# SamsungSAILMontreal/ghn3

Measured on AMD Instinct MI355X. Metric: predicted-params/sec (GHN fwd+bwd), ghn3xlm16, 256-node graphs, higher is better.
Workload: dtype f16; 1 GPU; ghn3xlm16 fwd+bwd, 1 synthetic 256-node graph(s) per GPU (seed 256000+), 86515016 predicted params per GPU, loss = sum of Frobenius norms of the predicted tensors; ghn_params=654365312, decoder_rows=1421, workspace_bytes=2436048640, zero_fill_bytes=2797339192, parallelism=dp1, index_mode=reference, loss=fused into the tile kernels

## Files before the change

ghn3_amd/csrc/elementwise.hip:

```cpp

#include "ghn3_internal.h"

#define MAX_DEGREE 100
#define MAX_INPUT_DIST 1000

__device__ __forceinline__ float wsum(float v) {
#pragma unroll
    for (int o = 32; o > 0; o >>= 1) v += __shfl_xor(v, o, 64);
    return v;
}

static int launch_ok(const char* what) {
    hipError_t e = hipGetLastError();
    if (e != hipSuccess) { ghn3_set_error("%s launch: %s", what, hipGetErrorString(e)); return GHN3_E_HIP; }
    return GHN3_OK;
}

__global__ __launch_bounds__(256) void graph_prologue_kernel(const int64_t* __restrict__ A, int* __restrict__ deg_in,
                                                             int* __restrict__ deg_out, int* __restrict__ dist0,
                                                             int* __restrict__ pair, int N, int V) {
    __shared__ int red[2][4];
    const int i = blockIdx.x, b = blockIdx.y;
    const int64_t* Ab = A + (size_t)b * N * N;
    int cnt_out = 0, cnt_in = 0;
// ... 703 lines not shown
                                                       float* __restrict__ b_parts) {
    extern __shared__ float tl[];
    float ss = 0.f, bm = 0.f;
    const int64_t di_raw = blocks[2 * (size_t)blockIdx.x];
    if (di_raw < 0) {
        const ghn3_tile_desc* D = desc + (~di_raw);
        const int64_t word = blocks[2 * (size_t)blockIdx.x + 1];
        const int a0 = (int)(word & 0xffffff), i0 = (int)(word >> 24);
        const int T1 = D->T[1], T3 = D->T[3], hw = D->T[2] * T3, E1 = D->E[1];
        const int ni = min(D->_pad, T1 - i0);
        const float* src = srcs.p[D->src_buf] + D->src_off + (int64_t)(a0 % D->E[0]) * D->S[0];
        const int n = ni * hw;
        const int S2 = (int)D->S[2], S3 = (int)D->S[3];
        const float inv_ni = 1.f / (float)ni, inv_t3 = 1.f / (float)T3;
        const bool vec = E1 == T1 && (ni & 3) == 0 && (S2 & 3) == 0 && (S3 & 3) == 0 &&
                         ((reinterpret_cast<uintptr_t>(src + i0)) & 15) == 0;
        if (vec) {
            const int ni4 = ni >> 2, n4 = ni4 * hw;
            const float inv_ni4 = 1.f / (float)ni4;
            constexpr int U = 4;
            for (int b0 = threadIdx.x; b0 < n4; b0 += 256 * U) {
                float4 v[U];
                int li[U];
#pragma unroll
                for (int u = 0; u < U; ++u) {
                    const int idx = b0 + 256 * u;
                    int pp = (int)((float)idx * inv_ni4);
                    int i4 = idx - pp * ni4;
                    if (i4 < 0) { i4 += ni4; --pp; } else if (i4 >= ni4) { i4 -= ni4; ++pp; }
                    int y = (int)((float)pp * inv_t3);
                    int x = pp - y * T3;
                    if (x < 0) { x += T3; --y; } else if (x >= T3) { x -= T3; ++y; }
                    li[u] = i4 * 4 * hw + pp;
                    v[u] = idx < n4 ? *reinterpret_cast<const float4*>(src + (int64_t)y * S2 + (int64_t)x * S3 + i0 + i4 * 4)
                                    : make_float4(0.f, 0.f, 0.f, 0.f);
                }
#pragma unroll
                for (int u = 0; u < U; ++u)
                    if (b0 + 256 * u < n4) {
                        tl[li[u]] = v[u].x; tl[li[u] + hw] = v[u].y; tl[li[u] + 2 * hw] = v[u].z; tl[li[u] + 3 * hw] = v[u].w;
                    }
            }
        } else {
            constexpr int U = 8;
            for (int b0 = threadIdx.x; b0 < n; b0 += 256 * U) {
                float v[U];
                int li[U];
#pragma unroll
                for (int u = 0; u < U; ++u) {
                    const int idx = b0 + 256 * u;
                    int pp = (int)((float)idx * inv_ni);
                    int i = idx - pp * ni;
                    if (i < 0) { i += ni; --pp; } else if (i >= ni) { i -= ni; ++pp; }
                    int y = (int)((float)pp * inv_t3);
                    int x = pp - y * T3;
                    if (x < 0) { x += T3; --y; } else if (x >= T3) { x -= T3; ++y; }
                    li[u] = i * hw + pp;
                    const int si = i0 + i;
                    v[u] = idx < n ? src[(int64_t)y * S2 + (int64_t)x * S3 + (E1 == T1 ? si : si % E1)] : 0.f;
                }
#pragma unroll
                for (int u = 0; u < U; ++u)
                    if (b0 + 256 * u < n) tl[li[u]] = v[u];
            }
        }
        __syncthreads();
        float* dst = flat + D->dst_off + ((int64_t)a0 * T1 + i0) * hw;
        const float scale = D->scale;
        const int nv = n & ~3;
        for (int j = threadIdx.x * 4; j < nv; j += 1024) {
            f4u o;
            o.x = tl[j] * scale; o.y = tl[j + 1] * scale; o.z = tl[j + 2] * scale; o.w = tl[j + 3] * scale;
            *reinterpret_cast<f4u*>(dst + j) = o;
            ss += (o.x * o.x + o.y * o.y) + (o.z * o.z + o.w * o.w);
            bm = fmaxf(fmaxf(bm, fmaxf(fabsf(o.x), fabsf(o.y))), fmaxf(fabsf(o.z), fabsf(o.w)));
        }
        for (int j = nv + threadIdx.x; j < n; j += 256) { const float o = tl[j] * scale; dst[j] = o; ss += o * o; bm = fmaxf(bm, fabsf(o)); }
        if (sq_parts) tile_block_sumsq(ss, bm, sq_parts, b_parts, D);
        return;
    }
    const int64_t di = di_raw;
    const unsigned start = (unsigned)blocks[2 * (size_t)blockIdx.x + 1];
    const ghn3_tile_desc* D = desc + di;
    const int T0 = D->T[0], T1 = D->T[1], T2 = D->T[2], T3 = D->T[3];
    const unsigned numel = (unsigned)T0 * T1 * T2 * T3;
    const unsigned end = min(numel, start + TILE_CHUNK);
    const float* src = srcs.p[D->src_buf] + D->src_off;
    float* dst = flat + D->dst_off;
    const int E0 = D->E[0], E1 = D->E[1], E2 = D->E[2], E3 = D->E[3];
    const bool w0 = E0 != T0, w1 = E1 != T1, w2 = E2 != T2, w3 = E3 != T3;
    const int S0 = (int)D->S[0], S1 = (int)D->S[1], S2 = (int)D->S[2], S3 = (int)D->S[3];
    const int mode = D->mode;
    const float scale = D->scale;
    Odo o;
    unsigned e = start + threadIdx.x;
    o.init(e, 256, T0, T1, T2, T3);
#pragma unroll 2
    for (; e < end; e += 256) {
        const int m0 = w0 ? o.d[0] % E0 : o.d[0];
        const int m1 = w1 ? o.d[1] % E1 : o.d[1];
        const int m2 = w2 ? o.d[2] % E2 : o.d[2];
        const int m3 = w3 ? o.d[3] % E3 : o.d[3];
        const int64_t so = (int64_t)m0 * S0 + (int64_t)m1 * S1 + (int64_t)m2 * S2 + (int64_t)m3 * S3;
        const float val = norm_apply(src[so], mode, scale);
        dst[e] = val;
        ss += val * val;
        bm = fmaxf(bm, fabsf(val));
        o.step();
    }
    if (sq_parts) tile_block_sumsq(ss, bm, sq_parts, b_parts, D);
}

int ghn3_tile_fwd(float* flat, const float* const* srcs, const ghn3_tile_desc* d_desc, int n_desc, int64_t total,
                  const int64_t* blocks, int lds_bytes, float* sq_parts, float* b_parts, hipStream_t s) {
    if (n_desc <= 0 || total <= 0) return GHN3_OK;
    SrcTable st;
    for (int i = 0; i < 6; ++i) st.p[i] = srcs[i];
    if (lds_bytes > 48 * 1024) {
        if (lds_bytes > 128 * 1024) { ghn3_set_error("tile_fwd: row blocks need %d bytes of LDS", lds_bytes); return GHN3_E_LIMIT; }
        hipFuncSetAttribute((const void*)tile_fwd_kernel, hipFuncAttributeMaxDynamicSharedMemorySize, lds_bytes);
    }
    hipLaunchKernelGGL(tile_fwd_kernel, dim3((unsigned)total), dim3(256), lds_bytes, s, flat, st, d_desc, blocks, sq_parts,
                       sq_parts ? b_parts : nullptr);
    return launch_ok("tile_fwd");
}

template <int U>
__device__ __forceinline__ void tile_bwd_gather(const float* __restrict__ p, int b0, int lim, f4u (&acc)[U]) {
#pragma unroll
    for (int u = 0; u < U; ++u) {
        const int j = b0 + 1024 * u;
        if (j + 4 <= lim) {
            acc[u] += *reinterpret_cast<const f4u*>(p + j);
        } else {
            if (j < lim) acc[u].x += p[j];
            if (j + 1 < lim) acc[u].y += p[j + 1];
            if (j + 2 < lim) acc[u].z += p[j + 2];
        }
    }
}
struct NormLoss { const float* out; const float* norms; const int* desc_seg; const float* g; };
struct H16 { const int64_t* tab; int bf16; };
__device__ __forceinline__ unsigned short h16_cast(float x, int bf16) {
    if (bf16) {
        const unsigned u = __float_as_uint(x);
        return (unsigned short)((u + 0x7fffu + ((u >> 16) & 1u)) >> 16);
    }
    return __builtin_bit_cast(unsigned short, (_Float16)x);
}
__device__ __forceinline__ int64_t h16_index(unsigned rel, unsigned ld32, unsigned ld16) {
    const unsigned r = rel / ld32;
    return (int64_t)r * ld16 + (rel - r * ld32);
}
__global__ __launch_bounds__(256) void tile_bwd_kernel(const float* __restrict__ dflat, SrcTable srcs, DstTable dsrcs,
                                                       const ghn3_tile_desc* __restrict__ desc,
                                                       const int64_t* __restrict__ blocks, float* __restrict__ amax,
                                                       NormLoss nl_, H16 h16) {
    extern __shared__ float tl[];
    float mx = 0.f;
    const int64_t di_raw = blocks[2 * (size_t)blockIdx.x];
    const int64_t di_any = di_raw < 0 ? ~di_raw : di_raw;
    float kn = 0.f;
    if (nl_.norms) {
        const float nrm = nl_.norms[nl_.desc_seg[di_any]];
        kn = nrm > 0.f ? nl_.g[0] / nrm : 0.f;
    }
    unsigned short* hdst = nullptr;
    unsigned hrel0 = 0, hld32 = 1, hld16 = 0;
    float hsc = 1.f;
    if (h16.tab) {
        const float bnd = nl_.norms[-1] * fabsf(nl_.g[0]);
        if (blockIdx.x == 0 && threadIdx.x == 0 && amax) amax[0] = bnd;
        const int64_t h = h16.tab[3 * di_any];
        if (h != INT64_MIN && desc[di_any].src_buf == 0) {
            hdst = reinterpret_cast<unsigned short*>(dsrcs.p[0]) + h;
            hrel0 = (unsigned)h16.tab[3 * di_any + 1];
            const int64_t lds_ = h16.tab[3 * di_any + 2];
            hld32 = (unsigned)(lds_ & 0xffffffff); hld16 = (unsigned)(lds_ >> 32);
            hsc = ghn3_pow2_scale(bnd);
        }
    }
    const float* __restrict__ outp = nl_.norms ? nl_.out + desc[di_any].dst_off : nullptr;
    if (di_raw < 0) {
        const ghn3_tile_desc* D = desc + (~di_raw);
        const int64_t word = blocks[2 * (size_t)blockIdx.x + 1];
        const int a0 = (int)(word & 0xffffff), i0 = (int)(word >> 24);
        const int T0 = D->T[0], T1 = D->T[1], T3 = D->T[3], hw = D->T[2] * T3;
        const int E0 = D->E[0], E1 = D->E[1], R1 = D->R[1];
        const int ni = min(D->_pad, R1 - i0);
        const int nl = max(0, min(ni, E1 - i0));
        float* dsrc = dsrcs.p[D->src_buf] + D->src_off + (int64_t)a0 * D->S[0] + i0;
        const float* g = dflat ? dflat + D->dst_off : nullptr;
        const bool live = a0 < E0 && nl > 0;
        if (live) {
            const int n = nl * hw;
            constexpr int U = 4;
            for (int b0 = threadIdx.x * 4; b0 < n; b0 += 1024 * U) {
                f4u acc[U], acc2[U];
#pragma unroll
                for (int u = 0; u < U; ++u) { acc[u] = f4u{0.f, 0.f, 0.f, 0.f}; acc2[u] = f4u{0.f, 0.f, 0.f, 0.f}; }
                for (int t0 = a0; t0 < T0; t0 += E0)
                    for (int r0 = 0; r0 + i0 < T1; r0 += E1) {
                        const int lim = min(nl, T1 - r0 - i0) * hw;
                        const int64_t go = ((int64_t)t0 * T1 + r0 + i0) * hw;
                        if (g) tile_bwd_gather<U>(g + go, b0, lim, acc);
                        if (outp) tile_bwd_gather<U>(outp + go, b0, lim, acc2);
                    }
                if (outp) {
#pragma unroll
                    for (int u = 0; u < U; ++u) {
                        acc[u].x += kn * acc2[u].x; acc[u].y += kn * acc2[u].y; acc[u].z += kn * acc2[u].z; acc[u].w += kn * acc2[u].w;
                    }
                }
#pragma unroll
                for (int u = 0; u < U; ++u) {
                    const int j = b0 + 1024 * u;
                    if (j + 4 <= n) {
                        *reinterpret_cast<float4*>(tl + j) = make_float4(acc[u].x, acc[u].y, acc[u].z, acc[u].w);
                    } else {
                        if (j < n) tl[j] = acc[u].x;
                        if (j + 1 < n) tl[j + 1] = acc[u].y;
                        if (j + 2 < n) tl[j + 2] = acc[u].z;
                    }
                }
            }
            __syncthreads();
        }
        const float scale = D->scale;
        const int S2 = (int)D->S[2], S3 = (int)D->S[3];
        const float inv_t3 = 1.f / (float)T3;
        if ((ni & 3) == 0 && (S2 & 3) == 0 && (S3 & 3) == 0 && (reinterpret_cast<uintptr_t>(dsrc) & 15) == 0) {
            const int ni4 = ni >> 2, nw4 = ni4 * hw;
            const float inv_ni4 = 1.f / (float)ni4;
            for (int idx = threadIdx.x; idx < nw4; idx += 256) {
                int pp = (int)((float)idx * inv_ni4);
                int i4 = idx - pp * ni4;
                if (i4 < 0) { i4 += ni4; --pp; } else if (i4 >= ni4) { i4 -= ni4; ++pp; }
                int y = (int)((float)pp * inv_t3);
                int x = pp - y * T3;
                if (x < 0) { x += T3; --y; } else if (x >= T3) { x -= T3; ++y; }
                const int i = i4 * 4;
                float4 val;
                val.x = (live && i < nl) ? tl[i * hw + pp] * scale : 0.f;
                val.y = (live && i + 1 < nl) ? tl[(i + 1) * hw + pp] * scale : 0.f;
                val.z = (live && i + 2 < nl) ? tl[(i + 2) * hw + pp] * scale : 0.f;
                val.w = (live && i + 3 < nl) ? tl[(i + 3) * hw + pp] * scale : 0.f;
                if (hdst) {
                    unsigned short* hp = hdst + h16_index(hrel0 + (unsigned)(a0 * (int)D->S[0] + i0 + y * S2 + x * S3 + i), hld32, hld16);
                    us4h o;
                    o[0] = h16_cast(val.x * hsc, h16.bf16); o[1] = h16_cast(val.y * hsc, h16.bf16);
                    o[2] = h16_cast(val.z * hsc, h16.bf16); o[3] = h16_cast(val.w * hsc, h16.bf16);
                    if ((reinterpret_cast<uintptr_t>(hp) & 7) == 0) *reinterpret_cast<us4h*>(hp) = o;
                    else { hp[0] = o[0]; hp[1] = o[1]; hp[2] = o[2]; hp[3] = o[3]; }
                    continue;
                }
                *reinterpret_cast<float4*>(dsrc + (int64_t)y * S2 + (int64_t)x * S3 + i) = val;
                mx = fmaxf(fmaxf(mx, fmaxf(fabsf(val.x), fabsf(val.y))), fmaxf(fabsf(val.z), fabsf(val.w)));
            }
        } else {
            const float inv_ni = 1.f / (float)ni;
            const int nw = ni * hw;
            for (int idx = threadIdx.x; idx < nw; idx += 256) {
                int pp = (int)((float)idx * inv_ni);
                int i = idx - pp * ni;
                if (i < 0) { i += ni; --pp; } else if (i >= ni) { i -= ni; ++pp; }
                int y = (int)((float)pp * inv_t3);
                int x = pp - y * T3;
                if (x < 0) { x += T3; --y; } else if (x >= T3) { x -= T3; ++y; }
                const float val = (live && i < nl) ? tl[i * hw + pp] * scale : 0.f;
                if (hdst) {
                    hdst[h16_index(hrel0 + (unsigned)(a0 * (int)D->S[0] + i0 + y * S2 + x * S3 + i), hld32, hld16)] = h16_cast(val * hsc, h16.bf16);
                    continue;
                }
                dsrc[(int64_t)y * S2 + (int64_t)x * S3 + i] = val;
                mx = fmaxf(mx, fabsf(val));
            }
        }
        if (amax && D->src_buf == 0 && !h16.tab) ghn3_atomic_amax(amax, mx);
        return;
    }
    const int64_t di = di_raw;
    const unsigned start = (unsigned)blocks[2 * (size_t)blockIdx.x + 1];
    const ghn3_tile_desc* D = desc + di;
    const int R0 = D->R[0], R1 = D->R[1], R2 = D->R[2], R3 = D->R[3];
    const unsigned numel = (unsigned)R0 * R1 * R2 * R3;
    const unsigned end = min(numel, start + TILE_CHUNK);
    const float* src = srcs.p[D->src_buf] + D->src_off;
    float* dsrc = dsrcs.p[D->src_buf] + D->src_off;
    const float* g = dflat ? dflat + D->dst_off : nullptr;
    const int T0 = D->T[0], T1 = D->T[1], T2 = D->T[2], T3 = D->T[3];
    const int E0 = D->E[0], E1 = D->E[1], E2 = D->E[2], E3 = D->E[3];
    const int S0 = (int)D->S[0], S1 = (int)D->S[1], S2 = (int)D->S[2], S3 = (int)D->S[3];
    const int mode = D->mode;
    const float scale = D->scale;
    Odo o;
    unsigned e = start + threadIdx.x;
    o.init(e, 256, R0, R2, R3, R1);
    for (; e < end; e += 256) {
        const int a0 = o.d[0], a2 = o.d[1], a3 = o.d[2], a1 = o.d[3];
        const int64_t so = (int64_t)a0 * S0 + (int64_t)a1 * S1 + (int64_t)a2 * S2 + (int64_t)a3 * S3;
        float acc = 0.f, acc2 = 0.f;
        if (a0 < E0 && a1 < E1 && a2 < E2 && a3 < E3) {
            for (int t0 = a0; t0 < T0; t0 += E0)
                for (int t1 = a1; t1 < T1; t1 += E1)
                    for (int t2 = a2; t2 < T2; t2 += E2)
                        for (int t3 = a3; t3 < T3; t3 += E3) {
                            const int64_t gi = (((int64_t)t0 * T1 + t1) * T2 + t2) * T3 + t3;
                            if (g) acc += g[gi];
                            if (outp) acc2 += outp[gi];
                        }
            acc = (acc + kn * acc2) * norm_grad(src[so], mode, scale);
        }
        if (hdst) hdst[h16_index(hrel0 + (unsigned)so, hld32, hld16)] = h16_cast(acc * hsc, h16.bf16);
        else dsrc[so] = acc;
        mx = fmaxf(mx, fabsf(acc));
        o.step();
    }
    if (amax && D->src_buf == 0 && !h16.tab) ghn3_atomic_amax(amax, mx);
}

int ghn3_tile_bwd(const float* dflat, const float* const* srcs, float* const* dsrcs, const ghn3_tile_desc* d_desc,
                  int n_desc, int64_t total, const int64_t* blocks, int lds_bytes, float* amax, const float* out,
                  const float* norms, const int* desc_seg, const float* gscale, const int64_t* h16_tab, int h16_bf16,
                  hipStream_t s) {
    if (n_desc <= 0 || total <= 0) return GHN3_OK;
    if (!dflat && !norms) { ghn3_set_error("tile_bwd: neither an upstream gradient nor the fused norm loss"); return GHN3_E_ARG; }
    if (norms && (!out || !desc_seg || !gscale)) { ghn3_set_error("tile_bwd: the fused norm loss needs out, the descriptor -> tensor table and g"); return GHN3_E_ARG; }
    if (h16_tab && (dflat || !norms || !amax)) { ghn3_set_error("tile_bwd: direct 16-bit tiles need the fused norm loss alone (no upstream gradient) and the amax slot"); return GHN3_E_ARG; }
    NormLoss nl{out, norms, desc_seg, gscale};
    H16 h16{h16_tab, h16_bf16};
    SrcTable st; DstTable dt;
    for (int i = 0; i < 6; ++i) { st.p[i] = srcs[i]; dt.p[i] = dsrcs[i]; }
    if (lds_bytes > 48 * 1024) {
        if (lds_bytes > 128 * 1024) { ghn3_set_error("tile_bwd: row blocks need %d bytes of LDS", lds_bytes); return GHN3_E_LIMIT; }
        hipFuncSetAttribute((const void*)tile_bwd_kernel, hipFuncAttributeMaxDynamicSharedMemorySize, lds_bytes);
    }
    hipLaunchKernelGGL(tile_bwd_kernel, dim3((unsigned)total), dim3(256), lds_bytes, s, dflat, st, dt, d_desc, blocks,
                       amax, nl, h16);
    return launch_ok("tile_bwd");
}

#define NORM_CHUNK 8192
__device__ __forceinline__ int first_segment_after(const int64_t* __restrict__ seg_off, int n_seg, int64_t pos) {
    int lo = 0, hi = n_seg;
    while (lo < hi) {
        const int mid = (lo + hi) >> 1;
        if (seg_off[2 * mid + 1] > pos) hi = mid; else lo = mid + 1;
    }
    return lo;
}
__global__ __launch_bounds__(256) void param_sq_kernel(const float* __restrict__ flat,
                                                       const int64_t* __restrict__ seg_off, float* __restrict__ norms,
                                                       int n_seg, const int* __restrict__ first_seg,
                                                       float* __restrict__ parts) {
    __shared__ float red[4];
    const int64_t w0 = (int64_t)blockIdx.x * NORM_CHUNK, w1 = w0 + NORM_CHUNK;
    const int sg0 = first_seg ? first_seg[blockIdx.x] : first_segment_after(seg_off, n_seg, w0);
    for (int sgm = sg0; sgm < n_seg && seg_off[2 * sgm] < w1; ++sgm) {
        const int64_t c0 = max(seg_off[2 * sgm], w0), c1 = min(seg_off[2 * sgm + 1], w1);
        float acc = 0.f;
        const int64_t a0 = (c0 + 3) & ~(int64_t)3, a1 = c1 & ~(int64_t)3;
        if (a0 < a1) {
            const float4* f4 = reinterpret_cast<const float4*>(flat + a0);
            const int64_t n4 = (a1 - a0) >> 2;
            for (int64_t q = threadIdx.x; q < n4; q += 256) {
                const float4 v = f4[q];
                acc += v.x * v.x + v.y * v.y + v.z * v.z + v.w * v.w;
            }
            for (int64_t e = c0 + threadIdx.x; e < a0; e += 256) { const float v = flat[e]; acc += v * v; }
            for (int64_t e = a1 + threadIdx.x; e < c1; e += 256) { const float v = flat[e]; acc += v * v; }
        } else {
            for (int64_t e = c0 + threadIdx.x; e < c1; e += 256) { const float v = flat[e]; acc += v * v; }
        }
        acc = wsum(acc);
        __syncthreads();
        if ((threadIdx.x & 63) == 0) red[threadIdx.x >> 6] = acc;
        __syncthreads();
        if (threadIdx.x == 0) {
            const float t = (red[0] + red[1]) + (red[2] + red[3]);
            if (parts && first_seg) parts[sg0 + (int64_t)blockIdx.x + (sgm - sg0)] = t;
            else if (t != 0.f) atomicAdd(&norms[sgm], t);
        }
    }
}
__global__ __launch_bounds__(256) void param_sqrt_kernel(float* __restrict__ norms, int n_seg,
                                                         const int64_t* __restrict__ seg_off,
                                                         const int* __restrict__ first_seg,
                                                         const float* __restrict__ parts) {
    const int i = blockIdx.x * 4 + (threadIdx.x >> 6), lane = threadIdx.x & 63;
    if (i >= n_seg) return;
    float sq = 0.f;
    if (parts && first_seg) {
        if (seg_off[2 * i + 1] > seg_off[2 * i]) {
            const int64_t b0 = seg_off[2 * i] / NORM_CHUNK, b1 = (seg_off[2 * i + 1] - 1) / NORM_CHUNK;
            for (int64_t b = b0 + lane; b <= b1; b += 64) sq += parts[b + i];
        }
        sq = wsum(sq);
    } else {
        sq = norms[i];
    }
    if (lane == 0) norms[i] = sqrtf(sq);
}
__global__ void param_loss_kernel(float* __restrict__ loss, const float* __restrict__ norms, int n_seg) {
    __shared__ float tot[256];
    float acc = 0.f;
    for (int i = threadIdx.x; i < n_seg; i += 256) acc += norms[i];
    tot[threadIdx.x] = acc;
    __syncthreads();
    if (threadIdx.x == 0) {
        float t = 0.f;
        for (int k = 0; k < 256; ++k) t += tot[k];
        loss[0] += t;
    }
}
__global__ __launch_bounds__(256) void param_norm_fin_kernel(float* __restrict__ norms, int n_seg,
                                                             const float* __restrict__ parts,
                                                             const int* __restrict__ first,
                                                             const float* __restrict__ b_parts, float* __restrict__ ratio) {
    const int i = blockIdx.x * 4 + (threadIdx.x >> 6), lane = threadIdx.x & 63;
    if (i >= n_seg) return;
    float sq = 0.f, bm = 0.f;
    for (int b = first[i] + lane; b < first[i + 1]; b += 64) { sq += parts[b]; if (b_parts) bm = fmaxf(bm, b_parts[b]); }
    sq = wsum(sq);
#pragma unroll
    for (int o = 32; o > 0; o >>= 1) bm = fmaxf(bm, __shfl_xor(bm, o, 64));
    if (lane == 0) {
        const float nrm = sqrtf(sq);
        norms[i] = nrm;
        if (ratio) ratio[i] = nrm > 0.f ? bm / nrm : 0.f;
    }
}
__global__ void param_loss_set_kernel(float* __restrict__ loss, const float* __restrict__ norms, int n_seg,
                                      const float* __restrict__ ratio, float* __restrict__ bound) {
    __shared__ float tot[256], mx[256];
    float acc = 0.f, m = 0.f;
    for (int i = threadIdx.x; i < n_seg; i += 256) { acc += norms[i]; if (ratio) m = fmaxf(m, ratio[i]); }
    tot[threadIdx.x] = acc;
    mx[threadIdx.x] = m;
    __syncthreads();
    if (threadIdx.x == 0) {
        float t = 0.f, b = 0.f;
        for (int k = 0; k < 256; ++k) { t += tot[k]; b = fmaxf(b, mx[k]); }
        loss[0] = t;
        if (bound) bound[0] = b;
    }
}
int ghn3_param_norm_fin(float* loss, float* norms, const float* parts, const int* first, int n_seg, const float* b_parts,
                        float* ratio, float* bound, hipStream_t s) {
    if (n_seg <= 0) return GHN3_OK;
    if (b_parts && !(ratio && bound)) { ghn3_set_error("PARAM_NORM_FIN: bound parts need the ratio scratch (r5) and the bound slot (r6)"); return GHN3_E_ARG; }
    if (!b_parts) ratio = nullptr, bound = nullptr;
    hipLaunchKernelGGL(param_norm_fin_kernel, dim3((n_seg + 3) / 4), dim3(256), 0, s, norms, n_seg, parts, first, b_parts, ratio);
    hipLaunchKernelGGL(param_loss_set_kernel, dim3(1), dim3(256), 0, s, loss, norms, n_seg, ratio, bound);
    return launch_ok("param_norm_fin");
}

int ghn3_param_norm_fwd(float* loss, const float* flat, const int64_t* seg_off, float* norms, int n_seg,
                        int64_t flat_numel, const int* first_seg, float* parts, hipStream_t s) {
    if (n_seg <= 0) return GHN3_OK;
    if (!(parts && first_seg)) hipMemsetAsync(norms, 0, sizeof(float) * n_seg, s);
    const int64_t blocks = (flat_numel + NORM_CHUNK - 1) / NORM_CHUNK;
    hipLaunchKernelGGL(param_sq_kernel, dim3((unsigned)blocks), dim3(256), 0, s, flat, seg_off, norms, n_seg,
                       first_seg, parts);
    hipLaunchKernelGGL(param_sqrt_kernel, dim3((n_seg + 3) / 4), dim3(256), 0, s, norms, n_seg, seg_off, first_seg, parts);
    hipLaunchKernelGGL(param_loss_kernel, dim3(1), dim3(256), 0, s, loss, norms, n_seg);
    return launch_ok("param_norm_fwd");
}
__global__ __launch_bounds__(256) void param_norm_bwd_kernel(float* __restrict__ dflat, const float* __restrict__ flat,
                                                             const int64_t* __restrict__ seg_off,
                                                             const float* __restrict__ norms, int n_seg, float g,
                                                             const int* __restrict__ first_seg) {
    const int64_t w0 = (int64_t)blockIdx.x * NORM_CHUNK, w1 = w0 + NORM_CHUNK;
    for (int sgm = first_seg ? first_seg[blockIdx.x] : first_segment_after(seg_off, n_seg, w0);
         sgm < n_seg && seg_off[2 * sgm] < w1; ++sgm) {
        const int64_t c0 = max(seg_off[2 * sgm], w0), c1 = min(seg_off[2 * sgm + 1], w1);
        const float nrm = norms[sgm];
        const float k = nrm > 0.f ? g / nrm : 0.f;
        const int64_t a0 = (c0 + 3) & ~(int64_t)3, a1 = c1 & ~(int64_t)3;
        if (a0 < a1) {
            const float4* f4 = reinterpret_cast<const float4*>(flat + a0);
            float4* d4 = reinterpret_cast<float4*>(dflat + a0);
            const int64_t n4 = (a1 - a0) >> 2;
            for (int64_t q = threadIdx.x; q < n4; q += 256) {
                float4 v = f4[q];
                v.x *= k; v.y *= k; v.z *= k; v.w *= k;
                d4[q] = v;
            }
            for (int64_t e = c0 + threadIdx.x; e < a0; e += 256) dflat[e] = flat[e] * k;
            for (int64_t e = a1 + threadIdx.x; e < c1; e += 256) dflat[e] = flat[e] * k;
        } else {
            for (int64_t e = c0 + threadIdx.x; e < c1; e += 256) dflat[e] = flat[e] * k;
// ... 901 lines not shown
```

ghn3_amd/csrc/ghn3_internal.h:

```cpp
#pragma once
#include <hip/hip_runtime.h>
#include <stdint.h>
#include "ghn3_hip.h"

struct GemmProbDev {
    const float* A; const float* B; float* C;
    const float* bias; const float* residual; const float* aux_in; float* aux_out;
    const int* a_gather; const int* b_gather; const int* c_gather;
    int M, N, K, lda, ldb, ldc;
    int a_q, a_s, b_q, b_s, c_q, c_s;
    int bias_q, bias_s, bias_stride;
    int act, dact, flags;
    float alpha;
    int tile_start;
    int tiles_m, tiles_n;
    int ksplit, k_chunk;
    int order;
    int kq, ks;
    const int* lim;
    int lim_kind;
    int xcd_cols;
    int pin;
    int pin_first, pin_count;
    int pin_end, pin_total;
    const float* alpha_amax;
    int ln_kind;
    float ln_eps;
    const float* ln_p[6];
    const void* B2;
    const int* mtab;
};


int ghn3_gemm_init();
int ghn3_gemm_launch(const GemmProbDev* d_probs, int n_probs, int total_tiles, int a_mode, int b_mode,
                     int tile, int ctype, hipStream_t stream);

int ghn3_gemm_h16d_launch(const GemmProbDev* d_probs, int n_probs, int total_tiles, int tile, int ctype, int grid_cap,
                          hipStream_t stream);
int ghn3_gemm_p8_init();
int ghn3_gemm_p8_launch(const GemmProbDev* d_probs, int n_probs, int total_tiles, int ctype, int grid_cap,
                        hipStream_t stream);
int ghn3_gemm_p8w_launch(const GemmProbDev* d_probs, int n_probs, int total_tiles, int ctype, int grid_cap,
                         hipStream_t stream);
int ghn3_gemm_p8d_launch(const GemmProbDev* d_probs, int n_probs, int total_tiles, int ctype, int grid_cap,
                         hipStream_t stream);
int ghn3_gemm_x3_init();
int ghn3_gemm_x3_tile(int code, int slice, int* bm, int* bn);
int ghn3_gemm_x3_launch(const GemmProbDev* d_probs, int n_probs, int total_tiles, int code, int slice,
                        hipStream_t stream);
int ghn3_gemm_x3s_init();
int ghn3_gemm_x3s_tile(int code, int K, int ln_kind, int* bm, int* bn);
int ghn3_gemm_x3s_launch(const GemmProbDev* d_probs, const GemmProbDev* h_probs, int n_probs, int total_tiles, int code, int K,
                         int ln_kind, hipStream_t stream);
int ghn3_gemm_wg_launch(const GemmProbDev* d_probs, int n_probs, int total_tiles, int grid_cap, int tile_edge, hipStream_t stream);
int ghn3_gemm_small_launch(const GemmProbDev* d_probs, int n_probs, int total_tiles, int a_mode, int b_mode, int with_ln,
                           hipStream_t stream);

int ghn3_attn_init();
int ghn3_attn_fwd(float* out, const float* qkv, const float* bias, float* P, const int* n_nodes,
                  int B, int N, int C, int H, hipStream_t s);
int ghn3_attn_bwd(float* dqkv, const float* dO, const float* qkv, const float* P, const float* O, float* amax_out,
                  float* dBias, const int* n_nodes, int B, int N, int C, int H, int general, hipStream_t s);

int ghn3_graph_prologue(const int64_t* A, int* deg_in, int* deg_out, int* dist0, int* pair,
                        int B, int N, int V, hipStream_t s);
int ghn3_embed_nodes(float* x, const int* node_type, const int* shape_idx, const int* n_nodes, const int* node_off,
                     const float* E_type, const float* E_ch, const float* E_sp, const float* E_in,
                     const float* E_out, const float* E_dist, const int* deg_in, const int* deg_out,
                     const int* dist0, int B, int N, int C, hipStream_t s);
int ghn3_embed_bwd(const float* dx, const int* node_type, const int* shape_idx, const int* n_nodes,
                   const int* node_off, float* dE_type, float* dE_ch, float* dE_sp, float* dE_in, float* dE_out,
                   float* dE_dist, const int* deg_in, const int* deg_out, const int* dist0,
                   int B, int N, int C, int n_type, int n_ch, int n_sp, hipStream_t s);
int ghn3_edge_hidden(float* hid, const float* Pfw, const float* Pbw, int V, int C, hipStream_t s);
int ghn3_edge_hidden_bwd(float* dPfw, float* dPbw, float* dhid, const float* hid, int V, int C, hipStream_t s);
int ghn3_bias_gather(float* bias, const float* T, const int* pair, int B, int N, int H, hipStream_t s);
int ghn3_bias_hist(float* dT, const float* dBias, const int* pair, int B, int N, int H, int V, void* scratch,
                   int have_amax, hipStream_t s);
int ghn3_rowset_colsum(float* out, const float* X, const void* sets, int n_sets, int O, int I, hipStream_t s);
int ghn3_layernorm_fwd(float* y, float* x, const float* g, const float* b, float* mean, float* rstd, const float* add,
                       int n_add, int64_t add_stride, int rows, int C, float eps, hipStream_t s);
int ghn3_layernorm_bwd(float* dx, float* dy, const float* x, const float* g, const float* mean,
                       const float* rstd, const float* res, const float* add, int n_add, int64_t add_stride, int rows,
                       int C, hipStream_t s);
int ghn3_ln_param_grad(float* dg, float* db, const float* dy, const float* x, const float* mean,
                       const float* rstd, int rows, int C, int accum, hipStream_t s);
int ghn3_ln_param_grad_batch(float* gbase, const float* abase, const int64_t* table, int n_items, int rows, int C,
                             hipStream_t s);
int ghn3_tile_fwd(float* flat, const float* const* srcs, const ghn3_tile_desc* d_desc, int n_desc,
                  int64_t total, const int64_t* blocks, int lds_bytes, float* sq_parts, float* b_parts, hipStream_t s);
int ghn3_tile_bwd(const float* dflat, const float* const* srcs, float* const* dsrcs,
                  const ghn3_tile_desc* d_desc, int n_desc, int64_t total, const int64_t* blocks, int lds_bytes,
                  float* amax, const float* out, const float* norms, const int* desc_seg, const float* gscale,
                  const int64_t* h16_tab, int h16_bf16, hipStream_t s);
int ghn3_param_norm_fin(float* loss, float* norms, const float* parts, const int* first, int n_seg, const float* b_parts,
                        float* ratio, float* bound, hipStream_t s);
int ghn3_param_norm_fwd(float* loss, const float* flat, const int64_t* seg_off, float* norms, int n_seg,
                        int64_t flat_numel, const int* first_seg, float* parts, hipStream_t s);
int ghn3_param_norm_bwd(float* dflat, const float* flat, const int64_t* seg_off, const float* norms, int n_seg,
                        float g, int64_t flat_numel, const int* first_seg, hipStream_t s);
int ghn3_colsum(float* out, const float* X, int M, int N, int ld, int q, int sdim, int stride, int accum,
                const int* gather, hipStream_t s);
int ghn3_rowseg_sum(float* out, const float* X, const int* seg_ptr, const int* idx, int rows, int C, int ldx,
                    int ldo, int accum, hipStream_t s);
int ghn3_add(float* dst, const float* src, int64_t n, hipStream_t s);
int ghn3_transpose32(float* dst, const float* src, int rows, int cols, int ld_src, int ld_dst, int batch, int64_t sb, int64_t db,
                     hipStream_t s);
int ghn3_wire_pack(void* dst, const void* src, int64_t n, int64_t n_pad, int reverse, hipStream_t s);
int ghn3_rank_reduce(void* out, const void* in, int64_t per, int W, int in16, int out16, float scale, hipStream_t s);
int ghn3_cast16(const float* src, void* dst, const ghn3_cast_desc* d_desc, int n_desc, int total_blocks, float* dbias,
                const float* amax, int grid_cap, hipStream_t s);
int ghn3_sumsq(float* out, const float* x, int64_t n, float* parts, int64_t skip_lo, int64_t skip_hi, const float* extra,
               int n_extra, hipStream_t s);
int ghn3_adamw(float* p, const float* g, float* m, float* v, int64_t n, const float* sumsq, float lr, float beta1,
               float beta2, float eps, float weight_decay, float bias_corr1, float bias_corr2, float max_norm,
               float inv_scale, hipStream_t s);
int ghn3_adamw_cast16(float* p, const float* g, float* m, float* v, void* dst, const ghn3_cast_desc* d_desc, int n_desc,
                      int total_blocks, const float* sumsq, float lr, float beta1, float beta2, float eps, float weight_decay,
                      float bias_corr1, float bias_corr2, float max_norm, float inv_scale, hipStream_t s);
int ghn3_adamw_s16(float* p, const float* g, void* m, void* v, int64_t n, const float* sumsq, float lr, float beta1,
                   float beta2, float eps, float weight_decay, float bias_corr1, float bias_corr2, float max_norm,
                   float inv_scale, float step, float seed, int64_t base, hipStream_t s);
int ghn3_adamw_s16_cast16(float* p, const float* g, void* m, void* v, void* dst, const ghn3_cast_desc* d_desc, int n_desc,
                          int total_blocks, const float* sumsq, float lr, float beta1, float beta2, float eps,
                          float weight_decay, float bias_corr1, float bias_corr2, float max_norm, float inv_scale, float step,
                          float seed, int64_t base, hipStream_t s);
int ghn3_dact(float* X, const float* aux, int M, int N, int ld, int dact, float* amax, const float* parts, int n_parts,
              int64_t part_stride, int rows_parts, hipStream_t s);

int ghn3_relu_fix(float* X, const float* U, const float* W, const float* bias, int rows, int cols, int ld, int K, int q,
                  int sdim, float tau_rel, hipStream_t s);

void ghn3_set_error(const char* fmt, ...);

#ifdef __HIPCC__
__device__ __forceinline__ int ghn3_amax_exp(float amax) {
    return (int)((__float_as_uint(amax) >> 23) & 0xff) - 127;
}
__device__ __forceinline__ float ghn3_pow2_scale(float amax) {
    const int e = ghn3_amax_exp(amax);
    if (!(amax > 0.f) || e < -100) return 1.f;
    return __uint_as_float((unsigned)(127 + 11 - e) << 23);
}
__device__ __forceinline__ float ghn3_pow2_inv_scale(float amax) {
    const int e = ghn3_amax_exp(amax);
    if (!(amax > 0.f) || e < -100) return 1.f;
    return __uint_as_float((unsigned)(127 - 11 + e) << 23);
}
__device__ __forceinline__ void ghn3_atomic_amax(float* slot, float v) {
#pragma unroll
    for (int o = 32; o > 0; o >>= 1) v = fmaxf(v, __shfl_xor(v, o, 64));
    if ((threadIdx.x & 63) == 0 && v > *reinterpret_cast<volatile float*>(slot))
        atomicMax(reinterpret_cast<int*>(slot), __float_as_int(v));
}
#endif
```

ghn3_amd/csrc/runtime.hip:

```cpp

#include "ghn3_internal.h"
#include <cstdarg>
#include <cstdio>
#include <cstring>
#include <vector>
#include <algorithm>

static thread_local char g_err[512] = "";

void ghn3_set_error(const char* fmt, ...) {
    va_list ap;
    va_start(ap, fmt);
    vsnprintf(g_err, sizeof(g_err), fmt, ap);
    va_end(ap);
}

extern "C" const char* ghn3_last_error(void) { return g_err; }
extern "C" int ghn3_abi_version(void) { return GHN3_ABI_VERSION; }

#define HIPCHK(expr)                                                                  \
    do {                                                                              \
        hipError_t e_ = (expr);                                                       \
        if (e_ != hipSuccess) {                                                       \
            ghn3_set_error("%s failed: %s", #expr, hipGetErrorString(e_));            \
            return GHN3_E_HIP;                                                        \
        }                                                                             \
    } while (0)

static const int kStageSlots = 16;

struct Launch { int a_mode, b_mode, tile, first, count, tiles, with_ln, max_slice; };

struct SlotCache {
    bool valid = false;
    uint64_t stamp = 0;
    int n_ops = 0, n_problems = 0, n_bufs = 0;
    std::vector<ghn3_op> ops;
    std::vector<ghn3_gemm_problem> problems;
    std::vector<void*> bufs;
    std::vector<std::vector<Launch>> launches;
    hipStream_t up_stream = nullptr;
};

struct ghn3_ctx {
    SlotCache* cache;
    uint64_t clock;
    uint64_t cache_hits, cache_misses;
    GemmProbDev* h_stage[kStageSlots];
    GemmProbDev* d_stage[kStageSlots];
    hipEvent_t ev[kStageSlots];
    bool ev_used[kStageSlots];
    size_t cap;
    int ctype;
    int profile;
    double ms[GHN3_OP_KIND_COUNT];
    int64_t launches[GHN3_OP_KIND_COUNT];
    hipEvent_t pe0, pe1;
    std::vector<hipEvent_t>* pool;
    std::vector<int>* pool_tag;
    size_t pool_used;
    double tag_ms[256];
    int64_t tag_n[256];
    hipStream_t side;
    hipEvent_t ev_fork, ev_join, ev_mark[4];
    bool side_enabled;
    bool side_pending;
    bool mark_set[4];
};

static int ctx_reserve(ghn3_ctx* c, size_t n) {
    if (n <= c->cap) return GHN3_OK;
    size_t cap = std::max<size_t>(n, 1024);
    for (int i = 0; i < kStageSlots; ++i) {
        if (c->ev_used[i]) { HIPCHK(hipEventSynchronize(c->ev[i])); c->ev_used[i] = false; }
        if (c->h_stage[i]) HIPCHK(hipHostFree(c->h_stage[i]));
        if (c->d_stage[i]) HIPCHK(hipFree(c->d_stage[i]));
        c->h_stage[i] = nullptr; c->d_stage[i] = nullptr;
        c->cache[i].valid = false;
        c->cache[i].stamp = 0;
        HIPCHK(hipHostMalloc((void**)&c->h_stage[i], cap * sizeof(GemmProbDev), hipHostMallocDefault));
        HIPCHK(hipMalloc((void**)&c->d_stage[i], cap * sizeof(GemmProbDev)));
    }
    c->cap = cap;
    return GHN3_OK;
}

extern "C" int ghn3_ctx_create(ghn3_ctx** out) {
    if (!out) return GHN3_E_ARG;
    int ndev = 0;
    HIPCHK(hipGetDeviceCount(&ndev));
    if (ndev <= 0) { ghn3_set_error("no HIP device"); return GHN3_E_HIP; }
    ghn3_ctx* c = new ghn3_ctx();
    memset(c, 0, sizeof(*c));
    c->pool = new std::vector<hipEvent_t>();
    c->pool_tag = new std::vector<int>();
    c->cache = new SlotCache[kStageSlots];
    for (int i = 0; i < kStageSlots; ++i) HIPCHK(hipEventCreateWithFlags(&c->ev[i], hipEventDisableTiming));
    HIPCHK(hipEventCreate(&c->pe0));
    HIPCHK(hipEventCreate(&c->pe1));
    {
        int least = 0, greatest = 0;
        HIPCHK(hipDeviceGetStreamPriorityRange(&least, &greatest));
        HIPCHK(hipStreamCreateWithPriority(&c->side, hipStreamNonBlocking, least));
    }
    HIPCHK(hipEventCreateWithFlags(&c->ev_fork, hipEventDisableTiming));
    HIPCHK(hipEventCreateWithFlags(&c->ev_join, hipEventDisableTiming));
    for (int i = 0; i < 4; ++i) HIPCHK(hipEventCreateWithFlags(&c->ev_mark[i], hipEventDisableTiming));
    c->side_enabled = !(getenv("GHN3_NO_SIDE_STREAM") && atoi(getenv("GHN3_NO_SIDE_STREAM")) != 0);
    int rc = ghn3_gemm_init();
    if (rc) return rc;
    rc = ghn3_attn_init();
    if (rc) return rc;
    rc = ghn3_gemm_x3_init();
    if (rc) return rc;
    rc = ghn3_gemm_x3s_init();
    if (rc) return rc;
    rc = ghn3_gemm_p8_init();
    if (rc) return rc;
    rc = ctx_reserve(c, 1024);
    if (rc) return rc;
    *out = c;
    return GHN3_OK;
}

extern "C" void ghn3_ctx_destroy(ghn3_ctx* c) {
    if (!c) return;
    for (int i = 0; i < kStageSlots; ++i) {
        if (c->ev_used[i]) hipEventSynchronize(c->ev[i]);
        if (c->h_stage[i]) hipHostFree(c->h_stage[i]);
        if (c->d_stage[i]) hipFree(c->d_stage[i]);
        hipEventDestroy(c->ev[i]);
    }
    hipEventDestroy(c->pe0);
    hipEventDestroy(c->pe1);
    hipStreamSynchronize(c->side);
    hipStreamDestroy(c->side);
    hipEventDestroy(c->ev_fork);
    for (int i = 0; i < 4; ++i) hipEventDestroy(c->ev_mark[i]);
    hipEventDestroy(c->ev_join);
    for (hipEvent_t e : *c->pool) hipEventDestroy(e);
    delete c->pool;
    delete c->pool_tag;
    delete[] c->cache;
    delete c;
}

extern "C" int ghn3_ctx_set_compute_type(ghn3_ctx* c, int ctype) {
    if (!c) return GHN3_E_NOCTX;
    if (ctype < 0 || ctype > 2) { ghn3_set_error("bad compute type %d", ctype); return GHN3_E_ARG; }
    c->ctype = ctype;
    return GHN3_OK;
}

extern "C" int ghn3_profile_enable(ghn3_ctx* c, int mode) {
    if (!c) return GHN3_E_NOCTX;
    c->profile = mode;
    return GHN3_OK;
}
static int drain_pool(ghn3_ctx* c) {
    for (size_t k = 0; k < c->pool_used; ++k) {
        hipEvent_t e0 = (*c->pool)[2 * k], e1 = (*c->pool)[2 * k + 1];
        HIPCHK(hipEventSynchronize(e1));
        float ms = 0.f;
        HIPCHK(hipEventElapsedTime(&ms, e0, e1));
        const int tag = (*c->pool_tag)[k] & 255;
        c->tag_ms[tag] += ms;
        c->tag_n[tag] += 1;
    }
    c->pool_used = 0;
    return GHN3_OK;
}
extern "C" int ghn3_profile_read(ghn3_ctx* c, double* ms, int64_t* launches, int reset) {
    if (!c) return GHN3_E_NOCTX;
    for (int i = 0; i < GHN3_OP_KIND_COUNT; ++i) {
        if (ms) ms[i] = c->ms[i];
        if (launches) launches[i] = c->launches[i];
        if (reset) { c->ms[i] = 0; c->launches[i] = 0; }
    }
    return GHN3_OK;
}
extern "C" int ghn3_profile_read_tags(ghn3_ctx* c, double* ms256, int64_t* n256, int reset) {
    if (!c) return GHN3_E_NOCTX;
    int rc = drain_pool(c);
    if (rc) return rc;
    for (int i = 0; i < 256; ++i) {
        if (ms256) ms256[i] = c->tag_ms[i];
        if (n256) n256[i] = c->tag_n[i];
        if (reset) { c->tag_ms[i] = 0; c->tag_n[i] = 0; }
    }
    return GHN3_OK;
}

struct Resolver {
    void* const* bufs; int n_bufs; bool bad;
    template <typename T> T* get(const ghn3_ref& r) {
        if (r.buf < 0) return nullptr;
        if (r.buf >= n_bufs || bufs[r.buf] == nullptr) { bad = true; return nullptr; }
        return reinterpret_cast<T*>(reinterpret_cast<char*>(bufs[r.buf]) + r.off);
    }
};

static int pick_tile(const ghn3_gemm_problem& p, int forced, int64_t op_t64) {
    if (p.flags & GHN3_GEMM_X3) {
        if (forced == 44 || forced == 45 || p.ln_kind)
            return (forced == 45 ? 7000 : 6000) + 100 * (p.ln_kind & 3) + ((p.K / 64) % 100);
        return 4000 + 10 * (((forced >= 40 && forced <= 42) ? forced : 40) - 40) + p.x3_slice / 64;
    }
    if (p.ln_kind) return 32;
    if (p.flags & GHN3_GEMM_OP16) {
        if (forced == 16 || forced == 24 || forced == 20 || forced == 25 || forced == 29 || forced == 30) return forced;
        if (forced == 28) {
            const bool kmap_ok = p.b_kq == 0 || p.b_kq % 64 == 0 || 64 % p.b_kq == 0;
            return (p.ksplit <= 1 && p.M >= 160 && (p.N & 3) == 0 && kmap_ok && p.a_gather.buf < 0 && p.b_gather.buf < 0 &&
                    p.c_gather.buf < 0) ? 28 : 16;
        }
        const int64_t t256 = (int64_t)((p.M + 255) / 256) * ((p.N + 255) / 256) * (p.ksplit > 1 ? p.ksplit : 1);
        const double eff = ((double)p.M / (((p.M + 255) / 256) * 256.0)) * ((double)p.N / (((p.N + 255) / 256) * 256.0));
        return (t256 >= 200 && eff >= 0.8) ? 24 : 16;
    }
    if (forced == 48 || forced == 49) {
        const bool ok = p.a_mode == GHN3_MODE_COL && p.b_mode == GHN3_MODE_COL && p.ksplit <= 1 && (p.M & 3) == 0 &&
                        (p.N & 3) == 0 && (p.ldc & 3) == 0 && (p.C.off & 15) == 0 && (p.lda & 3) == 0 && (p.ldb & 3) == 0 &&
                        (p.A.off & 15) == 0 && (p.B.off & 15) == 0 && p.a_gather.buf < 0 &&
                        p.b_gather.buf < 0 && p.c_gather.buf < 0 && !p.a_q && !p.b_q && !p.c_q && !p.bias_q &&
                        p.act == GHN3_ACT_NONE && p.dact == GHN3_DACT_NONE && p.residual.buf < 0 && p.aux_out.buf < 0 &&
                        (p.bias.buf < 0 || (p.flags & GHN3_GEMM_BIASGRAD));
        return ok ? forced : 64;
    }
    if (forced == 32 || forced == 64 || forced == 128) return forced;
    const double flops = 2.0 * p.M * p.N * (double)p.K;
    if (p.ksplit <= 1 && op_t64 <= 640 && flops <= 4e9 && p.K <= 8192) return 32;
    const int64_t t128 = (int64_t)((p.M + 127) / 128) * ((p.N + 127) / 128) * (p.ksplit > 1 ? p.ksplit : 1);
    if (p.M >= 96 && p.N >= 96 && t128 >= 192) return 128;
    return 64;
}

static inline bool is16(int tl) { return tl == 16 || tl == 24 || tl == 20 || tl == 25 || tl == 28 || tl == 29 || tl == 30; }

extern "C" int ghn3_run(ghn3_ctx* c, const ghn3_op* ops, int n_ops, const ghn3_gemm_problem* problems, int n_problems,
                        void* const* bufs, int n_bufs, void* stream_) {
    if (!c) return GHN3_E_NOCTX;
    if (n_ops < 0 || (n_ops > 0 && !ops) || n_bufs < 0) { ghn3_set_error("ghn3_run: bad arguments"); return GHN3_E_ARG; }
    hipStream_t stream = (hipStream_t)stream_;
    Resolver R{bufs, n_bufs, false};

    std::vector<std::vector<Launch>> fresh_launches;
    const std::vector<std::vector<Launch>>* launches = &fresh_launches;
    size_t need = 0;
    for (int k = 0; k < n_ops; ++k)
        if (ops[k].kind == GHN3_OP_GEMM) need += (size_t)ops[k].i[1];
    GemmProbDev* hs = nullptr; GemmProbDev* ds = nullptr;
    static const bool use_cache = !(getenv("GHN3_RUN_CACHE") && atoi(getenv("GHN3_RUN_CACHE")) == 0);
    int hit = -1;
    if (need > 0) {
        int rc = ctx_reserve(c, need);
        if (rc) return rc;
        if (n_problems < 0 || (n_problems > 0 && !problems)) { ghn3_set_error("ghn3_run: bad problem table"); return GHN3_E_ARG; }
        for (int i = 0; use_cache && i < kStageSlots && hit < 0; ++i) {
            const SlotCache& e = c->cache[i];
            if (e.valid && e.n_ops == n_ops && e.n_problems == n_problems && e.n_bufs == n_bufs &&
                memcmp(e.bufs.data(), bufs, (size_t)n_bufs * sizeof(void*)) == 0 &&
                memcmp(e.ops.data(), ops, (size_t)n_ops * sizeof(ghn3_op)) == 0 &&
                memcmp(e.problems.data(), problems, (size_t)n_problems * sizeof(ghn3_gemm_problem)) == 0)
                hit = i;
// ... 632 lines not shown
```

Before: 15.13 billion predicted-params/s.

## Compute tile backward from source tensors instead of re-reading the predicted output

Adds a templated tile backward path for the fused-norm-loss, direct-16-bit case. For mode-0 tiles it recomputes the gradient from the source decoder buffer (scaled value times the repeat count times g/norm) rather than gathering the large tiled output tensor. This avoids streaming the full predicted-parameter output back from memory. It adds closed-form repeat counts, vectorised 16-bit stores and an env switch that defaults on, at the cost of more complex indexing and float-based division tricks.

```diff
diff --git a/ghn3_amd/csrc/elementwise.hip b/ghn3_amd/csrc/elementwise.hip
--- a/ghn3_amd/csrc/elementwise.hip
+++ b/ghn3_amd/csrc/elementwise.hip
@@ -879,6 +879,167 @@
     const unsigned r = rel / ld32;
     return (int64_t)r * ld16 + (rel - r * ld32);
 }
+template <int V>
+__device__ __forceinline__ void h16_store(unsigned short* hp, const unsigned short (&o)[V]) {
+    if constexpr (V == 4) {
+        if ((reinterpret_cast<uintptr_t>(hp) & 7) == 0) { *reinterpret_cast<us4h*>(hp) = us4h{o[0], o[1], o[2], o[3]}; return; }
+    }
+#pragma unroll
+    for (int c = 0; c < V; ++c) hp[c] = o[c];
+}
+template <int V>
+__device__ __forceinline__ void load_v(const float* __restrict__ p, float (&v)[V]) {
+    if constexpr (V == 4) { const f4u t = *reinterpret_cast<const f4u*>(p); v[0] = t.x; v[1] = t.y; v[2] = t.z; v[3] = t.w; }
+    else v[0] = p[0];
+}
+static int g_tile_bwd_src = 1;
+int ghn3_elementwise_init() {
+    if (getenv("GHN3_TILE_BWD_SRC")) g_tile_bwd_src = atoi(getenv("GHN3_TILE_BWD_SRC")) != 0;
+    return GHN3_OK;
+}
+template <int V, int U>
+__device__ __forceinline__ void tile_bwd_rows_src(const float* __restrict__ sp, unsigned short* __restrict__ hdst, unsigned hbase,
+                                                  unsigned hld32, unsigned hld16, int bf16, int ni, int nl, int hw, int T3, int S2,
+                                                  int S3, bool live, int n_lo, int n_hi, int thr, float kn, float scale,
+                                                  float hsc) {
+    const int niv = ni / V, nw = niv * hw;
+    const float inv_niv = 1.f / (float)niv, inv_t3 = 1.f / (float)T3;
+    const unsigned r0 = hbase / hld32, c0 = hbase - r0 * hld32;
+    const bool lin = S2 == T3 * S3 && S3 == (int)hld32 && c0 + (unsigned)ni <= hld32;
+    int pp = (int)((float)threadIdx.x * inv_niv);
+    int iv = (int)threadIdx.x - pp * niv;
+    if (iv < 0) { iv += niv; --pp; } else if (iv >= niv) { iv -= niv; ++pp; }
+    int dq = (int)(256.f * inv_niv);
+    int dr = 256 - dq * niv;
+    if (dr < 0) { dr += niv; --dq; } else if (dr >= niv) { dr -= niv; ++dq; }
+    auto step = [&]() {
+        iv += dr; pp += dq;
+        if (iv >= niv) { iv -= niv; ++pp; }
+    };
+    auto offset = [&](int p, int i) {
+        if (lin) return p * S3 + i;
+        int y = (int)((float)p * inv_t3);
+        int x = p - y * T3;
+        if (x < 0) { x += T3; --y; } else if (x >= T3) { x -= T3; ++y; }
+        return y * S2 + x * S3 + i;
+    };
+    auto put = [&](int p, int i, const unsigned short (&o)[V]) {
+        const int64_t at = lin ? (int64_t)(r0 + (unsigned)p) * hld16 + (c0 + (unsigned)i)
+                               : h16_index(hbase + (unsigned)offset(p, i), hld32, hld16);
+        h16_store<V>(hdst + at, o);
+    };
+    if (!live) {
+        unsigned short z[V];
+#pragma unroll
+        for (int c = 0; c < V; ++c) z[c] = h16_cast(0.f * hsc, bf16);
+        for (int idx = threadIdx.x; idx < nw; idx += 256) {
+            put(pp, iv * V, z);
+            step();
+        }
+        return;
+    }
+    if (thr >= ni) { n_lo += n_hi; n_hi = 0; }
+    const int i_last = (nl - 1) / V * V;
+    for (int b0 = threadIdx.x; b0 < nw; b0 += 256 * U) {
+        float v[U][V], a[U][V];
+        int pp_[U], i_[U];
+#pragma unroll
+        for (int u = 0; u < U; ++u) {
+            pp_[u] = pp; i_[u] = iv * V;
+            step();
+        }
+#pragma unroll
+        for (int u = 0; u < U; ++u)
+            load_v<V>(sp + (b0 + 256 * u < nw ? offset(pp_[u], i_[u]) - max(i_[u] - i_last, 0) : 0), v[u]);
+#pragma unroll
+        for (int u = 0; u < U; ++u)
+#pragma unroll
+            for (int c = 0; c < V; ++c) { v[u][c] *= scale; a[u][c] = 0.f; }
+        for (int k = 0; k < n_lo; ++k)
+#pragma unroll
+            for (int u = 0; u < U; ++u)
+#pragma unroll
+                for (int c = 0; c < V; ++c) a[u][c] += v[u][c];
+        if (n_hi > 0) {
+#pragma unroll
+            for (int u = 0; u < U; ++u)
+#pragma unroll
+                for (int c = 0; c < V; ++c) v[u][c] = i_[u] + c < thr ? v[u][c] : 0.f;
+            for (int k = 0; k < n_hi; ++k)
+#pragma unroll
+                for (int u = 0; u < U; ++u)
+#pragma unroll
+                    for (int c = 0; c < V; ++c) a[u][c] += v[u][c];
+        }
+#pragma unroll
+        for (int u = 0; u < U; ++u) {
+            if (b0 + 256 * u >= nw) break;
+            unsigned short o[V];
+#pragma unroll
+            for (int c = 0; c < V; ++c) {
+                const float val = i_[u] + c < nl ? (0.f + kn * a[u][c]) * scale : 0.f;
+                o[c] = h16_cast(val * hsc, bf16);
+            }
+            put(pp_[u], i_[u], o);
+        }
+    }
+}
+template <int V>
+__device__ __forceinline__ void tile_bwd_elems_src(const ghn3_tile_desc* __restrict__ D, const float* __restrict__ src,
+                                                   unsigned short* __restrict__ hdst, unsigned hrel0, unsigned hld32,
+                                                   unsigned hld16, int bf16, unsigned start, unsigned end, float kn, float hsc) {
+    constexpr int U = V == 4 ? 2 : 4;
+    const int R0 = D->R[0], R1 = D->R[1], R2 = D->R[2], R3 = D->R[3];
+    const int T0 = D->T[0], T1 = D->T[1], T2 = D->T[2], T3 = D->T[3];
+    const int E0 = D->E[0], E1 = D->E[1], E2 = D->E[2], E3 = D->E[3];
+    const int S0 = (int)D->S[0], S1 = (int)D->S[1], S2 = (int)D->S[2], S3 = (int)D->S[3];
+    const float scale = D->scale;
+    const unsigned qend = end / V;
+    Odo o;
+    o.init(start / V + threadIdx.x, 256, R0, R2, R3, R1 / V);
+    for (unsigned q0 = start / V + threadIdx.x; q0 < qend; q0 += 256 * U) {
+        float v[U][V];
+        unsigned rel[U];
+        int a1_[U], n023[U];
+#pragma unroll
+        for (int u = 0; u < U; ++u) {
+            const int a0 = o.d[0], a2 = o.d[1], a3 = o.d[2], a1 = o.d[3] * V;
+            const bool valid = q0 + 256 * u < qend;
+            const int64_t so = (int64_t)a0 * S0 + (int64_t)a1 * S1 + (int64_t)a2 * S2 + (int64_t)a3 * S3;
+            rel[u] = hrel0 + (unsigned)so;
+            a1_[u] = a1;
+            int n = 0;
+            if (valid && a0 < E0 && a2 < E2 && a3 < E3) {
+                int c0 = 0, c2 = 0, c3 = 0;
+                for (int t = a0; t < T0; t += E0) ++c0;
+                for (int t = a2; t < T2; t += E2) ++c2;
+                for (int t = a3; t < T3; t += E3) ++c3;
+                n = c0 * c2 * c3;
+            }
+            n023[u] = n;
+            load_v<V>(src + (valid ? so : 0), v[u]);
+            o.step();
+        }
+#pragma unroll
+        for (int u = 0; u < U; ++u) {
+            if (q0 + 256 * u >= qend) break;
+            unsigned short h[V];
+#pragma unroll
+            for (int c = 0; c < V; ++c) {
+                const int a1 = a1_[u] + c;
+                int n = 0;
+                if (a1 < E1) for (int t = a1; t < T1; t += E1) n += n023[u];
+                const float val = norm_apply(v[u][c], 0, scale);
+                float acc2 = 0.f;
+                for (int k = 0; k < n; ++k) acc2 += val;
+                const float acc = n > 0 ? (0.f + kn * acc2) * norm_grad(v[u][c], 0, scale) : 0.f;
+                h[c] = h16_cast(acc * hsc, bf16);
+            }
+            h16_store<V>(hdst + h16_index(rel[u], hld32, hld16), h);
+        }
+    }
+}
+template <bool SRC>
 __global__ __launch_bounds__(256) void tile_bwd_kernel(const float* __restrict__ dflat, SrcTable srcs, DstTable dsrcs,
                                                        const ghn3_tile_desc* __restrict__ desc,
                                                        const int64_t* __restrict__ blocks, float* __restrict__ amax,
@@ -886,26 +1047,80 @@
     extern __shared__ float tl[];
     float mx = 0.f;
     const int64_t di_raw = blocks[2 * (size_t)blockIdx.x];
+    const int64_t blk_word = SRC ? blocks[2 * (size_t)blockIdx.x + 1] : 0;
     const int64_t di_any = di_raw < 0 ? ~di_raw : di_raw;
     float kn = 0.f;
-    if (nl_.norms) {
-        const float nrm = nl_.norms[nl_.desc_seg[di_any]];
-        kn = nrm > 0.f ? nl_.g[0] / nrm : 0.f;
-    }
     unsigned short* hdst = nullptr;
     unsigned hrel0 = 0, hld32 = 1, hld16 = 0;
     float hsc = 1.f;
-    if (h16.tab) {
-        const float bnd = nl_.norms[-1] * fabsf(nl_.g[0]);
-        if (blockIdx.x == 0 && threadIdx.x == 0 && amax) amax[0] = bnd;
-        const int64_t h = h16.tab[3 * di_any];
-        if (h != INT64_MIN && desc[di_any].src_buf == 0) {
+    ghn3_tile_desc dd;
+    if constexpr (SRC) {
+        dd = desc[di_any];
+        const int seg = nl_.desc_seg[di_any];
+        const int64_t h = h16.tab[3 * di_any], rel0 = h16.tab[3 * di_any + 1], lds_ = h16.tab[3 * di_any + 2];
+        const float gs = nl_.g[0], bnd = nl_.norms[-1] * fabsf(gs);
+        const float nrm = nl_.norms[seg];
+        kn = nrm > 0.f ? gs / nrm : 0.f;
+        if (blockIdx.x == 0 && threadIdx.x == 0) amax[0] = bnd;
+        if (h != INT64_MIN && dd.src_buf == 0) {
             hdst = reinterpret_cast<unsigned short*>(dsrcs.p[0]) + h;
-            hrel0 = (unsigned)h16.tab[3 * di_any + 1];
-            const int64_t lds_ = h16.tab[3 * di_any + 2];
+            hrel0 = (unsigned)rel0;
             hld32 = (unsigned)(lds_ & 0xffffffff); hld16 = (unsigned)(lds_ >> 32);
             hsc = ghn3_pow2_scale(bnd);
         }
+    } else {
+        if (nl_.norms) {
+            const float nrm = nl_.norms[nl_.desc_seg[di_any]];
+            kn = nrm > 0.f ? nl_.g[0] / nrm : 0.f;
+        }
+        if (h16.tab) {
+            const float bnd = nl_.norms[-1] * fabsf(nl_.g[0]);
+            if (blockIdx.x == 0 && threadIdx.x == 0 && amax) amax[0] = bnd;
+            const int64_t h = h16.tab[3 * di_any];
+            if (h != INT64_MIN && desc[di_any].src_buf == 0) {
+                hdst = reinterpret_cast<unsigned short*>(dsrcs.p[0]) + h;
+                hrel0 = (unsigned)h16.tab[3 * di_any + 1];
+                const int64_t lds_ = h16.tab[3 * di_any + 2];
+                hld32 = (unsigned)(lds_ & 0xffffffff); hld16 = (unsigned)(lds_ >> 32);
+                hsc = ghn3_pow2_scale(bnd);
+            }
+        }
+    }
+    bool src_local = false;
+    if constexpr (SRC) src_local = hdst && dd.mode == 0;
+    if (src_local && di_raw < 0) {
+        const int a0 = (int)(blk_word & 0xffffff), i0 = (int)(blk_word >> 24);
+        const int T0 = dd.T[0], T1 = dd.T[1], T3 = dd.T[3], hw = dd.T[2] * T3;
+        const int E0 = dd.E[0], E1 = dd.E[1];
+        const int S0 = (int)dd.S[0], S2 = (int)dd.S[2], S3 = (int)dd.S[3];
+        const int ni = min(dd._pad, dd.R[1] - i0);
+        const int nl = max(0, min(ni, E1 - i0));
+        const bool live = a0 < E0 && nl > 0;
+        const int cnt0 = live ? (T0 - a0 + E0 - 1) / E0 : 0;
+        const int c_hi = live ? max(0, (T1 - i0 + E1 - 1) / E1) : 0;
+        const int n_lo = cnt0 * max(c_hi - 1, 0), n_hi = c_hi > 0 ? cnt0 : 0;
+        const int thr = T1 - i0 - (c_hi - 1) * E1;
+        const float* sp = srcs.p[0] + dd.src_off + (int64_t)a0 * S0 + i0;
+        const float* dsrc = dsrcs.p[0] + dd.src_off + (int64_t)a0 * S0 + i0;
+        const unsigned hbase = hrel0 + (unsigned)(a0 * S0 + i0);
+        if ((ni & 3) == 0 && (S2 & 3) == 0 && (S3 & 3) == 0 && (reinterpret_cast<uintptr_t>(dsrc) & 15) == 0)
+            tile_bwd_rows_src<4, 4>(sp, hdst, hbase, hld32, hld16, h16.bf16, ni, nl, hw, T3, S2, S3, live, n_lo, n_hi, thr, kn,
+                                    dd.scale, hsc);
+        else
+            tile_bwd_rows_src<1, 4>(sp, hdst, hbase, hld32, hld16, h16.bf16, ni, nl, hw, T3, S2, S3, live, n_lo, n_hi, thr, kn,
+                                    dd.scale, hsc);
+        return;
+    }
+    if (src_local) {
+        const unsigned start = (unsigned)blk_word;
+        const unsigned numel = (unsigned)dd.R[0] * dd.R[1] * dd.R[2] * dd.R[3];
+        const unsigned end = min(numel, start + TILE_CHUNK);
+        const float* src = srcs.p[0] + dd.src_off;
+        if (dd.S[1] == 1 && (dd.R[1] & 3) == 0 && ((dd.S[0] | dd.S[2] | dd.S[3]) & 3) == 0 && (hrel0 & 3) == 0 && (hld32 & 3) == 0)
+            tile_bwd_elems_src<4>(&dd, src, hdst, hrel0, hld32, hld16, h16.bf16, start, end, kn, hsc);
+        else
+            tile_bwd_elems_src<1>(&dd, src, hdst, hrel0, hld32, hld16, h16.bf16, start, end, kn, hsc);
+        return;
     }
     const float* __restrict__ outp = nl_.norms ? nl_.out + desc[di_any].dst_off : nullptr;
     if (di_raw < 0) {
@@ -921,7 +1136,7 @@
         const bool live = a0 < E0 && nl > 0;
         if (live) {
             const int n = nl * hw;
-            constexpr int U = 4;
+            constexpr int U = SRC ? 1 : 4;
             for (int b0 = threadIdx.x * 4; b0 < n; b0 += 1024 * U) {
                 f4u acc[U], acc2[U];
 #pragma unroll
@@ -1058,12 +1273,12 @@
     H16 h16{h16_tab, h16_bf16};
     SrcTable st; DstTable dt;
     for (int i = 0; i < 6; ++i) { st.p[i] = srcs[i]; dt.p[i] = dsrcs[i]; }
+    const auto kernel = (h16_tab && g_tile_bwd_src) ? tile_bwd_kernel<true> : tile_bwd_kernel<false>;
     if (lds_bytes > 48 * 1024) {
         if (lds_bytes > 128 * 1024) { ghn3_set_error("tile_bwd: row blocks need %d bytes of LDS", lds_bytes); return GHN3_E_LIMIT; }
-        hipFuncSetAttribute((const void*)tile_bwd_kernel, hipFuncAttributeMaxDynamicSharedMemorySize, lds_bytes);
-    }
-    hipLaunchKernelGGL(tile_bwd_kernel, dim3((unsigned)total), dim3(256), lds_bytes, s, dflat, st, dt, d_desc, blocks,
-                       amax, nl, h16);
+        hipFuncSetAttribute((const void*)kernel, hipFuncAttributeMaxDynamicSharedMemorySize, lds_bytes);
+    }
+    hipLaunchKernelGGL(kernel, dim3((unsigned)total), dim3(256), lds_bytes, s, dflat, st, dt, d_desc, blocks, amax, nl, h16);
     return launch_ok("tile_bwd");
 }
 
diff --git a/ghn3_amd/csrc/ghn3_internal.h b/ghn3_amd/csrc/ghn3_internal.h
--- a/ghn3_amd/csrc/ghn3_internal.h
+++ b/ghn3_amd/csrc/ghn3_internal.h
@@ -88,6 +88,7 @@
                        const float* rstd, int rows, int C, int accum, hipStream_t s);
 int ghn3_ln_param_grad_batch(float* gbase, const float* abase, const int64_t* table, int n_items, int rows, int C,
                              hipStream_t s);
+int ghn3_elementwise_init();
 int ghn3_tile_fwd(float* flat, const float* const* srcs, const ghn3_tile_desc* d_desc, int n_desc,
                   int64_t total, const int64_t* blocks, int lds_bytes, float* sq_parts, float* b_parts, hipStream_t s);
 int ghn3_tile_bwd(const float* dflat, const float* const* srcs, float* const* dsrcs,
diff --git a/ghn3_amd/csrc/runtime.hip b/ghn3_amd/csrc/runtime.hip
--- a/ghn3_amd/csrc/runtime.hip
+++ b/ghn3_amd/csrc/runtime.hip
@@ -110,6 +110,8 @@
     int rc = ghn3_gemm_init();
     if (rc) return rc;
     rc = ghn3_attn_init();
+    if (rc) return rc;
+    rc = ghn3_elementwise_init();
     if (rc) return rc;
     rc = ghn3_gemm_x3_init();
     if (rc) return rc;
```

Result: no change. 15.12 billion predicted-params/s (-0.1%).
